# VictoriaMetrics/VictoriaMetrics

Measured on NVIDIA H100. Metric: rollup samples/sec (block decode + rate, raw samples decoded and scanned per second), higher is better.
Workload: dtype int64 codec -> f64 rollup

## Files before the change

victoriametrics_b200/csrc/api.cu:

```cuda
#include <cuda_runtime.h>
#include <cuda_fp16.h>
#include <stdarg.h>
#include <stdio.h>
#include <string.h>
#include <stdlib.h>

#include <algorithm>
#include <vector>

#include "common.cuh"
#include "decode.cu"
#include "rollup.cu"
#include "fused.cu"
#include "zstd.cu"
#include "marshal.inc"
#include "encode.cu"

static thread_local char g_err[512];
void vmb_set_error(const char* fmt, ...) {
    va_list ap;
    va_start(ap, fmt);
    vsnprintf(g_err, sizeof(g_err), fmt, ap);
    va_end(ap);
}
extern "C" const char* vmb_last_error(void) { return g_err; }
extern "C" int vmb_version(void) { return 100; }

#define CU(call)                                                                                   \
    do {                                                                                           \
        cudaError_t e_ = (call);                                                                   \
        if (e_ != cudaSuccess) {                                                                   \
            vmb_set_error("%s failed: %s (%s:%d)", #call, cudaGetErrorString(e_), __FILE__, __LINE__); \
            return VMB_ERR_CUDA;                                                                   \
        }                                                                                          \
    } while (0)

struct DevBuf {
    void* p = nullptr;
    size_t cap = 0;
    int reserve(size_t bytes) {
        if (bytes <= cap) return 0;
        if (p) cudaFree(p);
        p = nullptr;
        cap = 0;
        size_t want = bytes + (bytes >> 3) + 256;
        cudaError_t e = cudaMalloc(&p, want);
        if (e != cudaSuccess) {
            vmb_set_error("cudaMalloc(%zu) failed: %s", want, cudaGetErrorString(e));
            p = nullptr;
            return VMB_ERR_NOMEM;
        }
        cap = want;
        return 0;
    }
    void release() {
        if (p) cudaFree(p);
        p = nullptr;
        cap = 0;
    }
};

enum Stage { ST_ZSTD, ST_DECODE, ST_PREAMBLE, ST_ROLLUP, ST_AGGR, ST_FUSED, ST__COUNT };

#define FUSED_CHUNKS_DEFAULT 4u
#define FUSED_CHUNKS_MAX 64u

struct vmb_ctx {
    int device = 0;
    cudaStream_t stream = 0;
    uint64_t launches = 0;
    bool timing = false;
    float stage_ms[ST__COUNT] = {};
    cudaEvent_t ev[ST__COUNT] = {};
    DevBuf zseq;
    DevBuf zscratch, zlit, zstatus, zjobs, zws, args1, args2, rolled, counters, tmp_out, grp, mheap, mnext;
    DevBuf bail, sub_arrays;
    DevBuf enc_vals, enc_deltas, enc_out, enc_meta;
    DevBuf aggr_state, grp_ids;
    DevBuf oa_keys, oa_keys2, oa_cell, oa_meta;
    DevBuf cv_runs, cv_aux, cv_uniq;
    void* comm = nullptr;
    bool comm_owned = false;
    int comm_ranks = 1, comm_rank = 0;
    bool fused = true;
    uint32_t fused_chunks = 0;
    uint32_t fused_ctas_per_sm = 0;
    cudaStream_t zstream = nullptr;
    std::vector<cudaEvent_t> zev;
    int64_t dedup_interval = 0;
    struct vmb_series* col_cache = nullptr;
    void* h_pinned = nullptr;
    void* pipe = nullptr;
    void (*pipe_destroy)(void*) = nullptr;
};

struct vmb_blocks {
    vmb_ctx* ctx = nullptr;
    size_t nblocks = 0, nseries = 0;
    uint64_t rows = 0, compressed = 0, scratch_total = 0;
    uint64_t merge_rows = 0;
    uint64_t seq_total = 0;
    bool needs_lit = false;
    uint32_t n_huf = 0, n_gen = 0, n_bad = 0;
    uint8_t* d_arrays = nullptr;
    uint64_t* d_ser_merge_off = nullptr;
    vmb_block_desc* d_descs = nullptr;
    uint8_t* d_payload = nullptr;
    uint8_t* d_payload_alloc = nullptr;
    ColInfo* d_cols = nullptr;
    uint64_t* d_row_off = nullptr;
    uint32_t* d_huf_list = nullptr;
    uint32_t* d_gen_list = nullptr;
    uint32_t* d_bad_list = nullptr;
    uint32_t* d_ser_first = nullptr;
    uint32_t* d_ser_nblocks = nullptr;
    uint32_t* d_fused_list = nullptr;
    std::vector<uint32_t> h_fused, h_unfused, h_ser_first, h_ser_nblocks;
    std::vector<uint32_t> h_huf_upto;
    std::vector<vmb_block_desc> h_descs;
    std::vector<ColInfo> h_cols;
};

struct vmb_series {
    vmb_ctx* ctx = nullptr;
    size_t nseries = 0, nblocks = 0;
    uint64_t rows = 0;
    int64_t* d_ts = nullptr;
    double* d_vals = nullptr;
    SeriesMeta* d_meta = nullptr;
    uint32_t* d_blk_lo = nullptr;
    uint32_t* d_blk_hi = nullptr;
    int32_t* d_blk_status = nullptr;
    bool stale_dropped = false, resets_removed = false;
    uint32_t pre_applied = 0;
    bool rolled = false;
    uint32_t applied_mut = 0;
    int64_t applied_max_stale = 0;
    bool values_are_int = false;
};

static inline void count_launch(vmb_ctx* c, int n = 1) { c->launches += (uint64_t)n; }
static inline size_t al16(size_t x) { return (x + 15) & ~(size_t)15; }

extern "C" int vmb_ctx_create(int device, vmb_ctx** out) {
    if (!out) return VMB_ERR_INVALID_ARG;
    int ndev = 0;
    cudaError_t e = cudaGetDeviceCount(&ndev);
    if (e != cudaSuccess || ndev == 0) {
        vmb_set_error("no CUDA device available (%s): libvmb200 has no CPU fallback", cudaGetErrorString(e));
        return VMB_ERR_CUDA;
    }
    if (device < 0 || device >= ndev) {
        vmb_set_error("device %d out of range (%d devices)", device, ndev);
        return VMB_ERR_INVALID_ARG;
    }
    CU(cudaSetDevice(device));
    cudaDeviceProp prop;
    CU(cudaGetDeviceProperties(&prop, device));
    if (prop.major != 9 || prop.minor != 0) {
        vmb_set_error("device %d is sm_%d%d; libvmb200 is built for sm_90a (H100) only", device, prop.major, prop.minor);
        return VMB_ERR_CUDA;
    }
    vmb_ctx* c = new vmb_ctx();
    c->device = device;
    c->fused = getenv("VMB_NO_FUSED") == nullptr;
    if (const char* s = getenv("VMB_FUSED_CHUNKS")) {
        const long v = atol(s);
        c->fused_chunks = v < 1 ? 1u : (v > (long)FUSED_CHUNKS_MAX ? FUSED_CHUNKS_MAX : (uint32_t)v);
    }
    if (const char* s = getenv("VMB_FUSED_CTAS_PER_SM")) {
        const long v = atol(s);
        c->fused_ctas_per_sm = v < 1 ? 1u : (v > FU_CTAS_PER_SM ? (uint32_t)FU_CTAS_PER_SM : (uint32_t)v);
    }
    for (cudaEvent_t& e : c->ev) CU(cudaEventCreate(&e));
    CU(cudaHostAlloc(&c->h_pinned, 4096, cudaHostAllocDefault));
    *out = c;
    return VMB_OK;
}
extern "C" void vmb_series_free(vmb_series* s);
extern "C" int vmb_ctx_comm_destroy(vmb_ctx* ctx);
extern "C" void vmb_ctx_destroy(vmb_ctx* c) {
    if (!c) return;
    cudaSetDevice(c->device);
    cudaStreamSynchronize(c->stream);
    vmb_ctx_comm_destroy(c);
    if (c->col_cache) vmb_series_free(c->col_cache);
    c->col_cache = nullptr;
    DevBuf* bufs[] = {&c->zscratch, &c->zlit, &c->zstatus, &c->zjobs, &c->zws, &c->args1, &c->args2, &c->rolled,
                      &c->counters, &c->tmp_out, &c->grp, &c->mheap, &c->mnext, &c->zseq, &c->bail, &c->sub_arrays, &c->aggr_state, &c->grp_ids, &c->enc_vals, &c->enc_deltas, &c->enc_out, &c->enc_meta,
                      &c->oa_keys, &c->oa_keys2, &c->oa_cell, &c->oa_meta, &c->cv_runs, &c->cv_aux, &c->cv_uniq};
    for (DevBuf* b : bufs) b->release();
    for (cudaEvent_t e : c->ev)
        if (e) cudaEventDestroy(e);
    for (cudaEvent_t e : c->zev) cudaEventDestroy(e);
    if (c->zstream) cudaStreamDestroy(c->zstream);
    if (c->h_pinned) cudaFreeHost(c->h_pinned);
    if (c->pipe && c->pipe_destroy) c->pipe_destroy(c->pipe);
    delete c;
}
extern "C" int vmb_ctx_set_stream(vmb_ctx* c, void* stream) {
    if (!c) return VMB_ERR_INVALID_ARG;
    c->stream = (cudaStream_t)stream;
    return VMB_OK;
}
extern "C" int vmb_ctx_set_dedup_interval(vmb_ctx* c, int64_t interval_ms) {
    if (!c || interval_ms < 0) return VMB_ERR_INVALID_ARG;
    c->dedup_interval = interval_ms;
    return VMB_OK;
}
extern "C" int vmb_ctx_set_fused(vmb_ctx* c, int enable) {
    if (!c) return VMB_ERR_INVALID_ARG;
    c->fused = enable != 0;
    return VMB_OK;
}
extern "C" int vmb_ctx_synchronize(vmb_ctx* c) {
    if (!c) return VMB_ERR_INVALID_ARG;
    CU(cudaSetDevice(c->device));
    CU(cudaStreamSynchronize(c->stream));
    return VMB_OK;
}
extern "C" uint64_t vmb_ctx_launch_count(const vmb_ctx* c) { return c ? c->launches : 0; }
extern "C" float vmb_ctx_last_stage_ms(const vmb_ctx* c, int stage) {
    return (c && stage >= 0 && stage < ST__COUNT) ? c->stage_ms[stage] : 0.f;
}
extern "C" int vmb_ctx_enable_stage_timing(vmb_ctx* c, int enable) {
// ... 395 lines not shown
    for (size_t i = 0; i < nblocks; i++) {
        vmb_block_desc& d = descs[i];
        int rc = vmb_block_desc_from_header(&d, headers + i * 81, tsid);
        if (rc) return rc;
        if (d.ts_off > ts_len || d.ts_size > ts_len - d.ts_off || d.val_off > val_len || d.val_size > val_len - d.val_off) {
            vmb_set_error("block %zu references bytes outside the part files (timestamps [%llu, +%u) of %zu, values [%llu, +%u) of %zu)", i,
                          (unsigned long long)d.ts_off, d.ts_size, ts_len, (unsigned long long)d.val_off, d.val_size, val_len);
            return VMB_ERR_SHORT_SRC;
        }
        if (i && memcmp(tsid, prev_tsid, 24) != 0) series++;
        memcpy(prev_tsid, tsid, 24);
        d.series_idx = series;
        total += al16((size_t)d.ts_size) + al16((size_t)d.val_size);
    }
    std::vector<uint8_t> arena(total + 16);
    size_t pos = 0;
    for (size_t i = 0; i < nblocks; i++) {
        vmb_block_desc& d = descs[i];
        if (d.ts_size) memcpy(arena.data() + pos, timestamps_bin + d.ts_off, d.ts_size);
        d.ts_off = pos;
        pos += al16((size_t)d.ts_size);
        if (d.val_size) memcpy(arena.data() + pos, values_bin + d.val_off, d.val_size);
        d.val_off = pos;
        pos += al16((size_t)d.val_size);
    }
    return blocks_upload_impl(ctx, descs.data(), nblocks, arena.data(), pos, out, 0);
}

extern "C" void vmb_series_free(vmb_series* s) {
    if (!s) return;
    if (s->ctx) cudaSetDevice(s->ctx->device);
    cudaFree(s->d_ts);
    cudaFree(s->d_vals);
    cudaFree(s->d_meta);
    cudaFree(s->d_blk_lo);
    cudaFree(s->d_blk_hi);
    cudaFree(s->d_blk_status);
    delete s;
}
extern "C" size_t vmb_series_count(const vmb_series* s) { return s ? s->nseries : 0; }
extern "C" uint64_t vmb_series_rows(const vmb_series* s) { return s ? s->rows : 0; }

__global__ void k_set_status(int32_t* status, const uint32_t* list, uint32_t n, int32_t v) {
    uint32_t i = blockIdx.x * blockDim.x + threadIdx.x;
    if (i < n) status[list[i]] = v;
}

static void zstd_huf_range(vmb_ctx* ctx, const vmb_blocks* b, ZstdParams Z, uint32_t h0, uint32_t h1, cudaStream_t st) {
    if (h0 >= h1) return;
    Z.jobs = (HufJob*)ctx->zjobs.p + h0;
    Z.list = b->d_huf_list + h0;
    Z.count = h1 - h0;
    launch_zstd_prepare(Z, st);
    launch_huf_decode(Z, st);
    count_launch(ctx, 2);
    if (b->needs_lit) {
        launch_zstd_sequences(Z, st);
        count_launch(ctx, 2);
    }
}

static int run_zstd(vmb_ctx* ctx, const vmb_blocks* b, int32_t** d_zstatus_out, uint32_t huf_end = UINT32_MAX,
                    ZstdParams* Zrest = nullptr) {
    cudaStream_t st = ctx->stream;
    *d_zstatus_out = nullptr;
    if (b->n_huf + b->n_gen + b->n_bad == 0) return VMB_OK;
    int rc;
    if ((rc = ctx->zscratch.reserve(b->scratch_total + 64))) return rc;
    if ((rc = ctx->zstatus.reserve(2 * b->nblocks * sizeof(int32_t)))) return rc;
    int32_t* d_zstatus = (int32_t*)ctx->zstatus.p;
    CU(cudaMemsetAsync(d_zstatus, 0, 2 * b->nblocks * sizeof(int32_t), st));
    if (b->needs_lit && (rc = ctx->zlit.reserve(b->scratch_total + 64))) return rc;
    ZstdParams Z;
    memset(&Z, 0, sizeof(Z));
    Z.descs = b->d_descs;
    Z.cols = b->d_cols;
    Z.payload = b->d_payload;
    Z.scratch = (uint8_t*)ctx->zscratch.p;
    Z.lit = b->needs_lit ? (uint8_t*)ctx->zlit.p : nullptr;
    if (b->seq_total) {
        if ((rc = ctx->zseq.reserve(b->seq_total * 8))) return rc;
        Z.seq_rec = (unsigned long long*)ctx->zseq.p;
    }
    Z.status = d_zstatus;
    if (b->n_bad) {
        k_set_status<<<(b->n_bad + 127) / 128, 128, 0, st>>>(d_zstatus, b->d_bad_list, b->n_bad, VMB_ERR_ZSTD);
        count_launch(ctx);
    }
    const uint32_t ws_threads = VMB_SMS * 2u * 32u;
    if (b->needs_lit || b->n_gen) {
        if ((rc = ctx->zws.reserve((size_t)ws_threads * zstd_serial_ws_bytes()))) return rc;
        Z.ws = ctx->zws.p;
        Z.ws_count = ws_threads;
    }
    if (b->n_huf && (rc = ctx->zjobs.reserve((size_t)b->n_huf * sizeof(HufJob)))) return rc;
    if (Zrest) *Zrest = Z;
    zstd_huf_range(ctx, b, Z, 0, std::min(huf_end, b->n_huf), st);
    if (b->n_gen) {
        Z.list = b->d_gen_list;
        Z.count = b->n_gen;
        launch_zstd_serial(Z, 1, st);
        count_launch(ctx);
    }
    *d_zstatus_out = d_zstatus;
    return VMB_OK;
}

// ... 699 lines not shown
    CU(cudaStreamSynchronize(ctx->stream));
    return VMB_OK;
}

static int column_cache_view(vmb_ctx* ctx, const vmb_blocks* b, vmb_series* view) {
    vmb_series* c = ctx->col_cache;
    if (c && (c->rows < b->rows + b->merge_rows || c->nseries < b->nseries || c->nblocks < b->nblocks)) {
        vmb_series_free(c);
        ctx->col_cache = c = nullptr;
    }
    if (!c) {
        int rc = alloc_series_for(ctx, b, &c);
        if (rc) return rc;
        ctx->col_cache = c;
    }
    *view = *c;
    view->nseries = b->nseries;
    view->nblocks = b->nblocks;
    view->rows = b->rows + b->merge_rows;
    view->stale_dropped = view->resets_removed = view->rolled = false;
    view->pre_applied = 0;
    return 0;
}

static const size_t FUSED_SMEM = (sizeof(FusedSmem) + 15) & ~(size_t)15;
template <typename K>
static uint32_t fused_grid(K kernel) {
    int blocks_per_sm = 0;
    cudaFuncSetAttribute(kernel, cudaFuncAttributeMaxDynamicSharedMemorySize, (int)FUSED_SMEM);
    if (cudaOccupancyMaxActiveBlocksPerMultiprocessor(&blocks_per_sm, kernel, FU_THREADS, FUSED_SMEM) != cudaSuccess || blocks_per_sm < 1)
        blocks_per_sm = 1;
    if (blocks_per_sm > FU_CTAS_PER_SM) blocks_per_sm = FU_CTAS_PER_SM;
    return VMB_SMS * (uint32_t)blocks_per_sm;
}

extern "C" int vmb_fused_grid(void) {
    static const uint32_t grid = fused_grid(k_fused_rollup<VMB_RF_RATE>);
    return (int)grid;
}
extern "C" int vmb_fused_grid_chunked(void) {
    return (int)std::min<uint32_t>((uint32_t)vmb_fused_grid(), VMB_SMS * FU_CTAS_PER_SM_OVERLAP);
}

static uint32_t fused_chunks(const vmb_ctx* ctx, const vmb_blocks* b) {
    const size_t nf = b->h_fused.size();
    uint32_t C = ctx->fused_chunks ? ctx->fused_chunks : FUSED_CHUNKS_DEFAULT;
    if (C > nf) C = (uint32_t)nf;
    if (C <= 1 || b->n_huf == 0) return 1;
    return b->h_huf_upto[nf / C] < b->n_huf ? C : 1u;
}

static uint32_t fused_ctas_per_sm(const vmb_ctx* ctx, uint32_t C, const vmb_rollup_cfg* cfg) {
    if (ctx->fused_ctas_per_sm) return ctx->fused_ctas_per_sm;
    return C > 1 && cfg->func_id == VMB_RF_RATE ? FU_CTAS_PER_SM_OVERLAP : FU_CTAS_PER_SM;
}

static void launch_fused(const FusedParams& P, uint32_t ctas_per_sm, cudaStream_t st) {
    if (!P.nlist) return;
    const size_t smem0 = FUSED_SMEM;
#define FUSED_LAUNCH(KERNEL, SMEM)                                                                                \
    do {                                                                                                          \
        static const uint32_t grid0 = fused_grid(KERNEL);                                                         \
        uint32_t grid = std::min(grid0, VMB_SMS * ctas_per_sm);                                                   \
        if (grid > P.nlist) grid = P.nlist;                                                                       \
        KERNEL<<<grid, FU_THREADS, (SMEM), st>>>(P);                                                              \
    } while (0)
    switch (P.cfg.func_id) {
#define FUSED_CASE(F) case F: FUSED_LAUNCH((k_fused_rollup<F>), smem0); break;
        FUSED_CASE(VMB_RF_RATE)
        FUSED_CASE(VMB_RF_DELTA)
        FUSED_CASE(VMB_RF_AVG)
        FUSED_CASE(VMB_RF_MIN)
        FUSED_CASE(VMB_RF_MAX)
        FUSED_CASE(VMB_RF_SUM)
        FUSED_CASE(VMB_RF_COUNT)
        FUSED_CASE(VMB_RF_QUANTILE)
        FUSED_CASE(VMB_RF_DEFAULT_ROLLUP)
        FUSED_CASE(VMB_RF_IDERIV)
        FUSED_CASE(VMB_RF_IDELTA)
        FUSED_CASE(VMB_RF_LAST)
        FUSED_CASE(VMB_RF_FIRST)
        FUSED_CASE(VMB_RF_STDDEV)
        FUSED_CASE(VMB_RF_STDVAR)
        FUSED_CASE(VMB_RF_CHANGES)
        FUSED_CASE(VMB_RF_DERIV)
#undef FUSED_CASE
        default: FUSED_LAUNCH((k_fused_rollup<-1>), smem0); break;
    }
#undef FUSED_LAUNCH
}

static bool fused_enabled(const vmb_ctx* ctx, const vmb_blocks* b, const vmb_rollup_cfg* cfg) {
    return ctx->fused && !b->h_fused.empty() && ctx->dedup_interval == 0 && !(cfg->flags & VMB_RC_PRE_MASK);
}

static int run_unfused_subset(vmb_ctx* ctx, const vmb_blocks* b, const std::vector<uint32_t>& sub, int32_t* d_zstatus,
                              int64_t tr_min, int64_t tr_max, const vmb_rollup_cfg* cfg, int64_t points, double* d_out,
                              const Counters& c, bool dense_rows) {
    cudaStream_t st = ctx->stream;
    std::vector<vmb_block_desc> descs;
    std::vector<uint32_t> blk_map;
    BlocksPlan pl;
    for (size_t i = 0; i < sub.size(); i++) {
        const uint32_t fb = b->h_ser_first[sub[i]], nb = b->h_ser_nblocks[sub[i]];
        for (uint32_t k = 0; k < nb; k++) {
            vmb_block_desc d = b->h_descs[fb + k];
            d.series_idx = (uint32_t)i;
// ... 401 lines not shown
```

victoriametrics_b200/csrc/zstd.cu:

```cuda
#include "common.cuh"
#include <mutex>

namespace {

__device__ __forceinline__ int hb32(uint32_t v) { return 31 - __clz((int)v); }

struct BitR {
    const uint8_t* base;
    int pos;
    uint64_t buf;
    int cnt;
    long long left;

    __device__ __forceinline__ void refill() {
        uint32_t w;
        if (pos >= 4) {
            w = load_u32_unaligned(base + pos - 4);
            pos -= 4;
        } else {
            w = 0;
            for (int i = 0; i < pos; i++) w |= (uint32_t)base[i] << (8 * i);
            w = pos ? (w << (8 * (4 - pos))) : 0u;
            pos = 0;
        }
// ... 689 lines not shown
        }
        if (hdr + csize >= bsize) break;
        if (regen > ci.content_size) break;
        uint32_t ftab[64];
        short norm[256];
        unsigned short next[256];
        int tlog = 0;
        __align__(16) uint8_t nb_local[256];
        uint32_t used = huf_read_weights(nb_local, &tlog, blk + hdr, csize, ftab, norm, next);
        if (!used) break;
#pragma unroll
        for (int k = 0; k < 32; k++) ((uint64_t*)job->nbits)[k] = ((const uint64_t*)nb_local)[k];
        uint32_t lrem = csize - used;
        const uint8_t* lp = blk + hdr + used;
        if (streams == 1) {
            job->stream_size[0] = lrem;
            job->stream_size[1] = job->stream_size[2] = job->stream_size[3] = 0;
            job->src_off = (uint64_t)(lp - P.payload);
        } else {
            if (lrem < 6) break;
            uint32_t s1 = lp[0] | (lp[1] << 8), s2 = lp[2] | (lp[3] << 8), s3 = lp[4] | (lp[5] << 8);
            if (6 + s1 + s2 + s3 > lrem) break;
            uint32_t seg = (regen + 3) / 4;
            if (seg * 3 > regen) break;
            job->stream_size[0] = s1;
            job->stream_size[1] = s2;
            job->stream_size[2] = s3;
            job->stream_size[3] = lrem - 6 - s1 - s2 - s3;
            job->src_off = (uint64_t)(lp + 6 - P.payload);
        }
        job->regen_size = regen;
        job->table_log = (uint8_t)tlog;
        uint32_t seq_off = hdr + csize;
        job->seq_off = (uint32_t)(blk - src) + seq_off;
        job->seq_size = bsize - seq_off;
        bool has_seq = blk[seq_off] != 0;
        if (!has_seq && (job->seq_size != 1 || regen != ci.content_size)) break;
        if (has_seq && !P.lit) break;
        job->dst_is_lit = has_seq ? 1 : 0;
        job->seq_big = 0;
        job->dst_off = ci.scratch_off;
        job->nstreams = (uint8_t)streams;
        rc = 0;
    } while (0);
    P.status[col] = rc;
}

#define HUF_WARPS 2
#define HUF_FRAMES_PER_WARP 8
#define HUF_MAX_LOG 11
#define HUF_RING 16
#define HUF_FRAME_BYTES (256 + 64)
#define HUF_WARP_TABLE_BYTES (HUF_FRAMES_PER_WARP * HUF_FRAME_BYTES)
#define HUF_FBIAS 0x4B000000u

__global__ void __launch_bounds__(HUF_WARPS * 32) k_huf_decode(ZstdParams P) {
    extern __shared__ __align__(16) uint8_t s_smem[];
    const int lane = lane_id();
    const int warp = threadIdx.x >> 5;
    const uint32_t groups = (P.count + HUF_FRAMES_PER_WARP - 1) / HUF_FRAMES_PER_WARP;
    uint8_t* wtab = s_smem + (size_t)warp * HUF_WARP_TABLE_BYTES;
    uint32_t* wring = (uint32_t*)(s_smem + (size_t)HUF_WARPS * HUF_WARP_TABLE_BYTES) + (size_t)warp * HUF_RING * 32;
    for (uint32_t g = blockIdx.x * HUF_WARPS + warp; g < groups; g += gridDim.x * HUF_WARPS) {
        for (int f = 0; f < HUF_FRAMES_PER_WARP; f++) {
            uint32_t ji = g * HUF_FRAMES_PER_WARP + f;
            if (ji >= P.count) break;
            const HufJob* job = &P.jobs[ji];
            if (job->nstreams == 0) continue;
            const int log = job->table_log;
            uint8_t* perm = wtab + f * HUF_FRAME_BYTES;
            float* thr = (float*)(perm + 256);
            short* adj = (short*)(perm + 256 + 40);
            uint32_t nb[8];
            uint64_t packed = *(const uint64_t*)(job->nbits + lane * 8);
#pragma unroll
            for (int k = 0; k < 8; k++) nb[k] = (uint32_t)(packed >> (8 * k)) & 0xff;
            uint32_t start = 0;
            uint32_t rank = 0;
            if (lane < 10) thr[lane] = __uint_as_float(HUF_FBIAS);
            __syncwarp();
            for (int len = log; len >= 1; len--) {
                uint32_t mine = 0;
#pragma unroll
                for (int k = 0; k < 8; k++) mine += (nb[k] == (uint32_t)len);
                uint32_t inc = mine;
#pragma unroll
                for (int off = 1; off < 32; off <<= 1) {
                    uint32_t t = __shfl_up_sync(VMB_FULL, inc, off);
                    if (lane >= off) inc += t;
                }
                uint32_t tot = __shfl_sync(VMB_FULL, inc, 31);
                if (lane == 0) {
                    if (len <= 10) thr[len - 1] = __uint_as_float(HUF_FBIAS | start);
                    adj[len] = (short)((int)rank - (int)(start >> (HUF_MAX_LOG - len)));
                }
                uint32_t r = rank + inc - mine;
#pragma unroll
                for (int k = 0; k < 8; k++) {
                    if (nb[k] == (uint32_t)len) perm[r++ & 255u] = (uint8_t)(lane * 8 + k);
                }
                rank += tot;
                start += tot << (HUF_MAX_LOG - len);
            }
        }
        __syncwarp();
        {
            const int f = lane >> 2, s = lane & 3;
            uint32_t ji = g * HUF_FRAMES_PER_WARP + f;
            bool active = ji < P.count;
            const HufJob* job = active ? &P.jobs[ji] : nullptr;
            if (active && (job->nstreams == 0 || s >= job->nstreams)) active = false;
            bool ok = true;
            if (active) {
                const uint8_t* perm = wtab + f * HUF_FRAME_BYTES;
                const short* adj = (const short*)(perm + 256 + 40);
                __half2 th2[5];
                {
                    const float* tf = (const float*)(perm + 256);
#pragma unroll
                    for (int j = 0; j < 5; j++) {
                        const uint32_t a = __float_as_uint(tf[2 * j]) & 0x7fffffu, b = __float_as_uint(tf[2 * j + 1]) & 0x7fffffu;
                        th2[j] = __halves2half2(__ushort2half_rn((unsigned short)a), __ushort2half_rn((unsigned short)b));
                    }
                }
                uint32_t regen = job->regen_size;
                uint32_t seg = job->nstreams == 1 ? regen : (regen + 3) / 4;
                uint32_t count = job->nstreams == 1 ? regen : (s < 3 ? seg : regen - 3 * seg);
                uint64_t soff = job->src_off;
                for (int k = 0; k < s; k++) soff += job->stream_size[k];
                uint32_t slen = job->stream_size[s];
                uint8_t* dst = (job->dst_is_lit ? P.lit : P.scratch) + job->dst_off + (size_t)s * seg;
                const uint8_t* base = P.payload + soff;
                uint32_t last = slen ? base[slen - 1] : 0;
                if (count == 0) {
                } else if (slen == 0 || last == 0) {
                    ok = false;
                } else {
                    const uint32_t total_bits = (slen - 1) * 8 + (uint32_t)hb32(last);
                    const uint8_t* endp = base + slen - 1;
                    const uint4* blk = (const uint4*)((uintptr_t)endp & ~(uintptr_t)15);
                    const uint4* blk_min = (const uint4*)(((uintptr_t)base & ~(uintptr_t)15) - 32);
                    uint32_t* ring = wring + lane;
                    uint32_t wr = 0, rd = 0;
                    uint64_t buf;
                    int cnt;
                    {
                        uint4 q = *blk;
                        uint64_t qlo = ((uint64_t)q.y << 32) | q.x, qhi = ((uint64_t)q.w << 32) | q.z;
                        uint32_t nbytes = (uint32_t)((uintptr_t)endp & 15) + 1;
                        uint32_t drop = (16 - nbytes) * 8;
                        if (drop >= 64) { qhi = qlo; qlo = 0; drop -= 64; }
                        if (drop) { qhi = (qhi << drop) | (qlo >> (64 - drop)); qlo <<= drop; }
                        uint32_t r = nbytes & 3;
                        if (r == 0) r = 4;
                        buf = qhi & ~(~0ull >> (8 * r));
                        cnt = (int)(8 * r);
                        qhi = (qhi << (8 * r)) | (r == 8 ? 0 : (qlo >> (64 - 8 * r)));
                        qlo <<= (8 * r);
                        uint32_t nw = (nbytes - r) >> 2;
                        for (uint32_t k = 0; k < nw; k++) {
                            ring[(wr & (HUF_RING - 1)) * 32] = (uint32_t)(qhi >> 32);
                            wr++;
                            qhi = (qhi << 32) | (qlo >> 32);
                            qlo <<= 32;
                        }
                        int skip = 8 - hb32(last);
                        buf <<= skip;
                        cnt -= skip;
#pragma unroll
                        for (int k = 0; k < 3; k++) {
                            if (blk > blk_min) blk--;
                            uint4 b = *blk;
                            ring[((wr + 0) & (HUF_RING - 1)) * 32] = b.w;
                            ring[((wr + 1) & (HUF_RING - 1)) * 32] = b.z;
                            ring[((wr + 2) & (HUF_RING - 1)) * 32] = b.y;
                            ring[((wr + 3) & (HUF_RING - 1)) * 32] = b.x;
                            wr += 4;
                        }
                    }
                    const int cnt_init = cnt;
                    uint4 pendA = make_uint4(0, 0, 0, 0), pendB = make_uint4(0, 0, 0, 0);
                    bool hasA = false, hasB = false;
                    uint32_t cand = ring[(rd & (HUF_RING - 1)) * 32];
#define HUF_PHASE(pend, has)                                                               \
    do {                                                                                   \
        if (has) {            \
            ring[((wr + 0) & (HUF_RING - 1)) * 32] = pend.w;                               \
            ring[((wr + 1) & (HUF_RING - 1)) * 32] = pend.z;                               \
            ring[((wr + 2) & (HUF_RING - 1)) * 32] = pend.y;                               \
            ring[((wr + 3) & (HUF_RING - 1)) * 32] = pend.x;                               \
            wr += 4;                                                                       \
        }                                                                                  \
                   \
        has = (wr - rd) + 8u <= (uint32_t)HUF_RING;                                        \
        if (has) {                                                                         \
            if (blk > blk_min) blk--;                                                      \
            pend = *blk;                                                                   \
        }                                                                                  \
        cand = ring[(rd & (HUF_RING - 1)) * 32];  \
    } while (0)
#define HUF_REFILL()                                                                       \
    do {                                                                                   \
        if (cnt <= 32) {                                                                   \
            buf |= (uint64_t)cand << (32 - cnt);                                           \
            cnt += 32;                                                                     \
            rd++;                                                                          \
        }                                                                                  \
        cand = ring[(rd & (HUF_RING - 1)) * 32];                                           \
    } while (0)
#define HUF_LT(k) __hlt2(vv_, th2[k])
#define HUF_SYM(outv, shift)                                                               \
    do {                                                                                   \
        const uint32_t v_ = (uint32_t)(buf >> 53);                                         \
        const __half2 vv_ = __half2half2(__ushort2half_rn((unsigned short)v_));            \
                  \
        const __half2 c_ = __hadd2(__hadd2(__hadd2(HUF_LT(0), HUF_LT(1)), __hadd2(HUF_LT(2), HUF_LT(3))), HUF_LT(4)); \
        const uint32_t nb_ = 1u + (uint32_t)__half2ushort_rz(__hadd(__low2half(c_), __high2half(c_))); \
        buf <<= nb_;                                                                       \
        cnt -= (int)nb_;                                                                   \
        const uint32_t sym_ = perm[((v_ >> (HUF_MAX_LOG - nb_)) + (uint32_t)(int)adj[nb_]) & 255u]; \
        outv |= sym_ << (shift);                                                           \
    } while (0)
                    uint32_t i = 0;
                    while (i < count && (((uintptr_t)(dst + i)) & 15)) {
                        HUF_REFILL();
                        uint32_t o = 0;
                        HUF_SYM(o, 0);
                        dst[i++] = (uint8_t)o;
                    }
                    for (; i + 16 <= count; i += 16) {
                        uint32_t o[4];
                        HUF_PHASE(pendA, hasA);
#pragma unroll
                        for (int q = 0; q < 2; q++) {
                            o[q] = 0;
                            HUF_REFILL();
                            HUF_SYM(o[q], 0);
                            HUF_SYM(o[q], 8);
                            HUF_REFILL();
                            HUF_SYM(o[q], 16);
                            HUF_SYM(o[q], 24);
                        }
                        HUF_PHASE(pendB, hasB);
#pragma unroll
                        for (int q = 2; q < 4; q++) {
                            o[q] = 0;
                            HUF_REFILL();
                            HUF_SYM(o[q], 0);
                            HUF_SYM(o[q], 8);
                            HUF_REFILL();
                            HUF_SYM(o[q], 16);
                            HUF_SYM(o[q], 24);
                        }
                        *(uint4*)(dst + i) = make_uint4(o[0], o[1], o[2], o[3]);
                    }
                    if (i < count) {
                        HUF_PHASE(pendA, hasA);
                        HUF_PHASE(pendB, hasB);
                        hasA = hasB = false;
                    }
                    for (; i < count; i++) {
                        HUF_REFILL();
                        uint32_t o = 0;
                        HUF_SYM(o, 0);
                        dst[i] = (uint8_t)o;
                    }
#undef HUF_PHASE
#undef HUF_REFILL
#undef HUF_SYM
#undef HUF_LT
                    ok = (long long)cnt_init + 32ll * (long long)rd - (long long)cnt == (long long)total_bits;
                }
            }
            uint32_t bad = __ballot_sync(VMB_FULL, active && !ok);
            if (ji < P.count && s == 0 && ((bad >> (f * 4)) & 0xf)) P.status[P.jobs[ji].col] = VMB_ERR_ZSTD;
        }
        __syncwarp();
    }
}

#define SEQ_G 4
#define SEQ_FPW (32 / SEQ_G)
#define SEQ_WARPS 1
#define SEQ_REC(ll, ml, of) (((unsigned long long)(ll) << 44) | ((unsigned long long)(ml) << 24) | (unsigned long long)(of))
#define SEQ_REC_LL(r) ((uint32_t)((r) >> 44))
#define SEQ_REC_ML(r) ((uint32_t)((r) >> 24) & 0xfffffu)
#define SEQ_REC_OF(r) ((uint32_t)(r) & 0xffffffu)
template <int LLC, int MLC, int OFC>
struct SeqTablesT {
    unsigned short ll_nb[LLC], ml_nb[MLC], of_nb[OFC];
    uint8_t ll_sym[LLC], ml_sym[MLC], of_sym[OFC];
};

__device__ bool fse_build_packed(uint8_t* sym, unsigned short* nbbase, const short* norm, int nsym, int log, unsigned short* next) {
    const int size = 1 << log;
    int high = size - 1;
    for (int s = 0; s < nsym; s++) {
        if (norm[s] == -1) {
            sym[high--] = (uint8_t)s;
            next[s] = 1;
        } else {
            next[s] = (unsigned short)norm[s];
        }
    }
    const int step = (size >> 1) + (size >> 3) + 3, mask = size - 1;
    int pos = 0;
    for (int s = 0; s < nsym; s++) {
        for (int i = 0; i < norm[s]; i++) {
            sym[pos] = (uint8_t)s;
            do {
                pos = (pos + step) & mask;
            } while (pos > high);
        }
    }
    if (pos != 0) return false;
    for (int i = 0; i < size; i++) {
        const uint32_t s = sym[i];
        const uint32_t ns = next[s]++;
        const int nb = log - hb32(ns);
        nbbase[i] = (unsigned short)(((uint32_t)nb << 12) | ((ns << nb) - (uint32_t)size));
    }
    return true;
}

#define SEQ_DEF_LL 0
#define SEQ_DEF_OF 64
#define SEQ_DEF_ML 96
__device__ unsigned short g_seq_def_nb[160];
__device__ uint8_t g_seq_def_sym[160];
__global__ void k_zstd_seq_defaults() {
    if (blockIdx.x || threadIdx.x) return;
// ... 372 lines not shown
                __syncwarp();
            }
            o_base += __shfl_sync(VMB_FULL, so, 31);
            l_base += __shfl_sync(VMB_FULL, sl, 31);
        }
        warp_copy(out + o_base, lits + l_base, job->regen_size - l_base, lane);
        __syncwarp();
    }
}

__global__ void k_zstd_serial(ZstdParams P, int mode) {
    uint32_t tid = blockIdx.x * blockDim.x + threadIdx.x;
    if (tid >= P.ws_count) return;
    SerialWs* ws = (SerialWs*)P.ws + tid;
    for (uint32_t i = tid; i < P.count; i += P.ws_count) {
        if (mode == 0) {
            const HufJob* job = &P.jobs[i];
            if (job->nstreams == 0 || !job->dst_is_lit) continue;
            uint32_t col = job->col;
            if (P.status[col]) continue;
            const ColInfo ci = P.cols[col];
            const uint8_t* src;
            uint32_t len;
            col_src(P, col, &src, &len);
            ws->have_ll = ws->have_ml = ws->have_of = 0;
            ws->rep[0] = 1;
            ws->rep[1] = 4;
            ws->rep[2] = 8;
            long long o = run_sequences(ws, P.scratch + ci.scratch_off, 0, ci.content_size, P.lit + ci.scratch_off,
                                        job->regen_size, src + job->seq_off, job->seq_size);
            if (o != (long long)ci.content_size) P.status[col] = VMB_ERR_ZSTD;
        } else {
            uint32_t col = P.list[i];
            const ColInfo ci = P.cols[col];
            const uint8_t* src;
            uint32_t len;
            col_src(P, col, &src, &len);
            const long long o = P.lit ? decode_frame_serial(ws, P.scratch + ci.scratch_off, ci.content_size,
                                                            P.lit + ci.scratch_off, src, len)
                                      : -1;
            P.status[col] = o >= 0 ? 0 : VMB_ERR_ZSTD;
            if (o >= 0 && o != (long long)ci.content_size) P.cols[col].content_size = (uint32_t)o;
        }
    }
}

size_t zstd_serial_ws_bytes() { return sizeof(SerialWs); }

void launch_zstd_prepare(const ZstdParams& P, cudaStream_t st) {
    if (!P.count) return;
    k_zstd_prepare<<<(P.count + 63) / 64, 64, 0, st>>>(P);
}

void launch_huf_decode(const ZstdParams& P, cudaStream_t st) {
    if (!P.count) return;
    constexpr size_t smem = (size_t)HUF_WARPS * HUF_WARP_TABLE_BYTES + (size_t)HUF_WARPS * HUF_RING * 32 * sizeof(uint32_t);
    static_assert(smem <= 48 * 1024, "k_huf_decode would need cudaFuncAttributeMaxDynamicSharedMemorySize");
    uint32_t groups = (P.count + HUF_FRAMES_PER_WARP - 1) / HUF_FRAMES_PER_WARP;
    uint32_t grid = (groups + HUF_WARPS - 1) / HUF_WARPS;
    if (grid > VMB_SMS * 12u) grid = VMB_SMS * 12u;
    k_huf_decode<<<grid, HUF_WARPS * 32, smem, st>>>(P);
}

void launch_zstd_sequences(const ZstdParams& P, cudaStream_t st) {
    if (!P.count || !P.ws_count || !P.seq_rec) return;
    const uint32_t per_cta = SEQ_WARPS * SEQ_FPW;
    const uint64_t slots = (uint64_t)P.ws_count * sizeof(SerialWs) / sizeof(SeqWs);
    uint64_t groups = P.count < slots ? P.count : slots;
    uint32_t grid = (uint32_t)((groups + per_cta - 1) / per_cta);
    if ((uint64_t)grid * per_cta > slots) grid = (uint32_t)(slots / per_cta);
    if (grid == 0) grid = 1;
    {
        static std::mutex mu;
        static bool built[64] = {};
        int dev = 0;
        cudaGetDevice(&dev);
        std::lock_guard<std::mutex> lk(mu);
        if (!built[dev & 63]) {
            k_zstd_seq_defaults<<<1, 32, 0, st>>>();
            if (cudaStreamSynchronize(st) == cudaSuccess) built[dev & 63] = true;
        }
    }
    k_zstd_seq_decode<false><<<grid, SEQ_WARPS * 32, 0, st>>>(P);
    k_zstd_seq_decode<true><<<grid, SEQ_WARPS * 32, 0, st>>>(P);
    uint32_t xgrid = (P.count + SEQX_WARPS - 1) / SEQX_WARPS;
    if (xgrid > VMB_SMS * 64u) xgrid = VMB_SMS * 64u;
    k_zstd_seq_exec<<<xgrid, SEQX_WARPS * 32, 0, st>>>(P);
}

void launch_zstd_serial(const ZstdParams& P, int mode, cudaStream_t st) {
    if (!P.count || !P.ws_count) return;
    uint32_t threads = P.ws_count < P.count ? P.ws_count : P.count;
    k_zstd_serial<<<(threads + 31) / 32, 32, 0, st>>>(P, mode);
}


static bool zstd_content_bound_host(const FrameHdr& h, const uint8_t* src, uint32_t len, unsigned long long* bound) {
    unsigned long long b = 0;
    uint32_t pos = h.hdr_size;
    for (;;) {
        if (pos + 3 > len) return false;
        const uint32_t bh = src[pos] | ((uint32_t)src[pos + 1] << 8) | ((uint32_t)src[pos + 2] << 16);
        pos += 3;
        const uint32_t bsize = bh >> 3, type = (bh >> 1) & 3;
        if (type == 3) return false;
        const uint32_t stored = type == 1 ? 1u : bsize;
        if ((unsigned long long)pos + stored > len) return false;
        pos += stored;
        b += type == 2 ? h.block_max : bsize;
        if (bh & 1) break;
    }
    *bound = b;
    return true;
}

// ... 66 lines not shown
```

Baseline: 61.96 billion.

## Stage Huffman decode output in shared memory for coalesced warp stores

The Huffman decode body now writes each lane's 16-byte output chunks into a per-warp shared-memory staging ring. When the ring fills, the warp cooperatively flushes it so consecutive lanes write consecutive 16-byte pieces of the same stream, instead of each lane scattering its own uint4 stores. The change also lowers the default fused chunk count from 4 to 2, always uses the normal fused CTAs-per-SM, and adds an env knob for Huffman CTAs per SM. Compile-time experiment flags (phase timers, L1 no-allocate loads, integer threshold compare) are added but off by default. The cost is more shared memory per CTA and extra warp votes and shuffles in the loop.

```diff
diff --git a/victoriametrics_b200/csrc/api.cu b/victoriametrics_b200/csrc/api.cu
--- a/victoriametrics_b200/csrc/api.cu
+++ b/victoriametrics_b200/csrc/api.cu
@@ -62,7 +62,7 @@
 
 enum Stage { ST_ZSTD, ST_DECODE, ST_PREAMBLE, ST_ROLLUP, ST_AGGR, ST_FUSED, ST__COUNT };
 
-#define FUSED_CHUNKS_DEFAULT 4u
+#define FUSED_CHUNKS_DEFAULT 2u
 #define FUSED_CHUNKS_MAX 64u
 
 struct vmb_ctx {
@@ -85,6 +85,7 @@
     bool fused = true;
     uint32_t fused_chunks = 0;
     uint32_t fused_ctas_per_sm = 0;
+    uint32_t huf_ctas_per_sm = 0;
     cudaStream_t zstream = nullptr;
     std::vector<cudaEvent_t> zev;
     int64_t dedup_interval = 0;
@@ -171,6 +172,10 @@
     if (const char* s = getenv("VMB_FUSED_CTAS_PER_SM")) {
         const long v = atol(s);
         c->fused_ctas_per_sm = v < 1 ? 1u : (v > FU_CTAS_PER_SM ? (uint32_t)FU_CTAS_PER_SM : (uint32_t)v);
+    }
+    if (const char* s = getenv("VMB_HUF_CTAS_PER_SM")) {
+        const long v = atol(s);
+        c->huf_ctas_per_sm = v < 1 ? 1u : (v > 32 ? 32u : (uint32_t)v);
     }
     for (cudaEvent_t& e : c->ev) CU(cudaEventCreate(&e));
     CU(cudaHostAlloc(&c->h_pinned, 4096, cudaHostAllocDefault));
@@ -672,7 +677,7 @@
     Z.list = b->d_huf_list + h0;
     Z.count = h1 - h0;
     launch_zstd_prepare(Z, st);
-    launch_huf_decode(Z, st);
+    launch_huf_decode(Z, ctx->huf_ctas_per_sm, st);
     count_launch(ctx, 2);
     if (b->needs_lit) {
         launch_zstd_sequences(Z, st);
@@ -1478,7 +1483,9 @@
 
 static uint32_t fused_ctas_per_sm(const vmb_ctx* ctx, uint32_t C, const vmb_rollup_cfg* cfg) {
     if (ctx->fused_ctas_per_sm) return ctx->fused_ctas_per_sm;
-    return C > 1 && cfg->func_id == VMB_RF_RATE ? FU_CTAS_PER_SM_OVERLAP : FU_CTAS_PER_SM;
+    (void)C;
+    (void)cfg;
+    return FU_CTAS_PER_SM;
 }
 
 static void launch_fused(const FusedParams& P, uint32_t ctas_per_sm, cudaStream_t st) {
diff --git a/victoriametrics_b200/csrc/zstd.cu b/victoriametrics_b200/csrc/zstd.cu
--- a/victoriametrics_b200/csrc/zstd.cu
+++ b/victoriametrics_b200/csrc/zstd.cu
@@ -765,7 +765,49 @@
 #define HUF_RING 16
 #define HUF_FRAME_BYTES (256 + 64)
 #define HUF_WARP_TABLE_BYTES (HUF_FRAMES_PER_WARP * HUF_FRAME_BYTES)
+#ifndef HUF_STAGE
+#define HUF_STAGE 8
+#endif
+#define HUF_STAGE_SLOT(q, l) ((q) * 32 + ((l) ^ ((q) * (8 / HUF_STAGE))))
 #define HUF_FBIAS 0x4B000000u
+#define HUF_CTAS_PER_SM 12u
+
+#ifndef VMB_HUF_EXP
+#define VMB_HUF_EXP 0
+#endif
+#define HUF_EXP_STORE 1
+#define HUF_EXP_LOOKUP 2
+#define HUF_EXP_CONVERT 4
+#define HUF_EXP_INPUT 8
+#define HUF_EXP_L1 16
+#define HUF_EXP_PHASES 32
+#define HUF_EXP_CARVEOUT 64
+#define HUF_EXP(bit) ((VMB_HUF_EXP & (bit)) != 0)
+enum { HUF_PH_BUILD, HUF_PH_PRIME, HUF_PH_HEAD, HUF_PH_BODY, HUF_PH_TAIL, HUF_PH_N, HUF_PH_SYMS = HUF_PH_N, HUF_PH_SLOTS };
+#if HUF_EXP(HUF_EXP_PHASES)
+__device__ unsigned long long huf_phase_cyc[HUF_PH_SLOTS];
+#define HUF_PH(k)                                                                              \
+    do {                                                                                       \
+        const long long ph_c = clock64();                                                      \
+        ph[(k)] += (unsigned long long)(ph_c - ph_t);                                          \
+        ph_t = ph_c;                                                                           \
+    } while (0)
+#else
+#define HUF_PH(k) \
+    do {          \
+    } while (0)
+#endif
+
+__device__ __forceinline__ uint4 huf_ldg(const uint4* p) {
+    if (HUF_EXP(HUF_EXP_L1)) {
+        uint4 r;
+        asm volatile("ld.global.nc.L1::no_allocate.v4.u32 {%0,%1,%2,%3}, [%4];"
+                     : "=r"(r.x), "=r"(r.y), "=r"(r.z), "=r"(r.w)
+                     : "l"(p));
+        return r;
+    }
+    return *p;
+}
 
 __global__ void __launch_bounds__(HUF_WARPS * 32) k_huf_decode(ZstdParams P) {
     extern __shared__ __align__(16) uint8_t s_smem[];
@@ -774,6 +816,10 @@
     const uint32_t groups = (P.count + HUF_FRAMES_PER_WARP - 1) / HUF_FRAMES_PER_WARP;
     uint8_t* wtab = s_smem + (size_t)warp * HUF_WARP_TABLE_BYTES;
     uint32_t* wring = (uint32_t*)(s_smem + (size_t)HUF_WARPS * HUF_WARP_TABLE_BYTES) + (size_t)warp * HUF_RING * 32;
+#if HUF_EXP(HUF_EXP_PHASES)
+    unsigned long long ph[HUF_PH_SLOTS] = {};
+    long long ph_t = clock64();
+#endif
     for (uint32_t g = blockIdx.x * HUF_WARPS + warp; g < groups; g += gridDim.x * HUF_WARPS) {
         for (int f = 0; f < HUF_FRAMES_PER_WARP; f++) {
             uint32_t ji = g * HUF_FRAMES_PER_WARP + f;
@@ -817,6 +863,7 @@
             }
         }
         __syncwarp();
+        HUF_PH(HUF_PH_BUILD);
         {
             const int f = lane >> 2, s = lane & 3;
             uint32_t ji = g * HUF_FRAMES_PER_WARP + f;
@@ -824,10 +871,22 @@
             const HufJob* job = active ? &P.jobs[ji] : nullptr;
             if (active && (job->nstreams == 0 || s >= job->nstreams)) active = false;
             bool ok = true;
+            bool live = false;
+            const uint8_t* perm = wtab + f * HUF_FRAME_BYTES;
+            const short* adj = (const short*)(perm + 256 + 40);
+            __half2 th2[5];
+            uint32_t th_i[5] = {0, 0, 0, 0, 0};
+            uint32_t count = 0, total_bits = 0, wr = 0, rd = 0, cand = 0, i = 0;
+            uint8_t* dst = nullptr;
+            const uint4* blk = nullptr;
+            const uint4* blk_min = nullptr;
+            uint32_t* ring = wring + lane;
+            uint64_t buf = 0;
+            int cnt = 0, cnt_init = 0;
+            uint4 pendA = make_uint4(0, 0, 0, 0), pendB = make_uint4(0, 0, 0, 0);
+            bool hasA = false, hasB = false;
+            uint4 xo = make_uint4(0, 0, 0, 0);
             if (active) {
-                const uint8_t* perm = wtab + f * HUF_FRAME_BYTES;
-                const short* adj = (const short*)(perm + 256 + 40);
-                __half2 th2[5];
                 {
                     const float* tf = (const float*)(perm + 256);
 #pragma unroll
@@ -836,27 +895,31 @@
                         th2[j] = __halves2half2(__ushort2half_rn((unsigned short)a), __ushort2half_rn((unsigned short)b));
                     }
                 }
+                if (HUF_EXP(HUF_EXP_CONVERT)) {
+                    const float* tf = (const float*)(perm + 256);
+#pragma unroll
+                    for (int j = 0; j < 5; j++)
+                        th_i[j] = ((0x1000u + (__float_as_uint(tf[2 * j + 1]) & 0x7fffffu)) << 16) |
+                                  (0x1000u + (__float_as_uint(tf[2 * j]) & 0x7fffffu));
+                }
                 uint32_t regen = job->regen_size;
                 uint32_t seg = job->nstreams == 1 ? regen : (regen + 3) / 4;
-                uint32_t count = job->nstreams == 1 ? regen : (s < 3 ? seg : regen - 3 * seg);
+                count = job->nstreams == 1 ? regen : (s < 3 ? seg : regen - 3 * seg);
                 uint64_t soff = job->src_off;
                 for (int k = 0; k < s; k++) soff += job->stream_size[k];
                 uint32_t slen = job->stream_size[s];
-                uint8_t* dst = (job->dst_is_lit ? P.lit : P.scratch) + job->dst_off + (size_t)s * seg;
+                dst = (job->dst_is_lit ? P.lit : P.scratch) + job->dst_off + (size_t)s * seg;
                 const uint8_t* base = P.payload + soff;
                 uint32_t last = slen ? base[slen - 1] : 0;
                 if (count == 0) {
                 } else if (slen == 0 || last == 0) {
                     ok = false;
                 } else {
-                    const uint32_t total_bits = (slen - 1) * 8 + (uint32_t)hb32(last);
+                    live = true;
+                    total_bits = (slen - 1) * 8 + (uint32_t)hb32(last);
                     const uint8_t* endp = base + slen - 1;
-                    const uint4* blk = (const uint4*)((uintptr_t)endp & ~(uintptr_t)15);
-                    const uint4* blk_min = (const uint4*)(((uintptr_t)base & ~(uintptr_t)15) - 32);
-                    uint32_t* ring = wring + lane;
-                    uint32_t wr = 0, rd = 0;
-                    uint64_t buf;
-                    int cnt;
+                    blk = (const uint4*)((uintptr_t)endp & ~(uintptr_t)15);
+                    blk_min = (const uint4*)(((uintptr_t)base & ~(uintptr_t)15) - 32);
                     {
                         uint4 q = *blk;
                         uint64_t qlo = ((uint64_t)q.y << 32) | q.x, qhi = ((uint64_t)q.w << 32) | q.z;
@@ -883,7 +946,7 @@
 #pragma unroll
                         for (int k = 0; k < 3; k++) {
                             if (blk > blk_min) blk--;
-                            uint4 b = *blk;
+                            uint4 b = huf_ldg(blk);
                             ring[((wr + 0) & (HUF_RING - 1)) * 32] = b.w;
                             ring[((wr + 1) & (HUF_RING - 1)) * 32] = b.z;
                             ring[((wr + 2) & (HUF_RING - 1)) * 32] = b.y;
@@ -891,10 +954,8 @@
                             wr += 4;
                         }
                     }
-                    const int cnt_init = cnt;
-                    uint4 pendA = make_uint4(0, 0, 0, 0), pendB = make_uint4(0, 0, 0, 0);
-                    bool hasA = false, hasB = false;
-                    uint32_t cand = ring[(rd & (HUF_RING - 1)) * 32];
+                    cnt_init = cnt;
+                    cand = ring[(rd & (HUF_RING - 1)) * 32];
 #define HUF_PHASE(pend, has)                                                               \
     do {                                                                                   \
         if (has) {            \
@@ -908,7 +969,8 @@
         has = (wr - rd) + 8u <= (uint32_t)HUF_RING;                                        \
         if (has) {                                                                         \
             if (blk > blk_min) blk--;                                                      \
-            pend = *blk;                                                                   \
+            if (HUF_EXP(HUF_EXP_INPUT)) pend = make_uint4(rd, wr, (uint32_t)cnt, (uint32_t)(uintptr_t)blk); \
+            else pend = huf_ldg(blk);                                                      \
         }                                                                                  \
         cand = ring[(rd & (HUF_RING - 1)) * 32];  \
     } while (0)
@@ -922,26 +984,44 @@
         cand = ring[(rd & (HUF_RING - 1)) * 32];                                           \
     } while (0)
 #define HUF_LT(k) __hlt2(vv_, th2[k])
+#define HUF_LTI(j) ((th_i[j] - v1_) & 0x10001000u)
 #define HUF_SYM(outv, shift)                                                               \
     do {                                                                                   \
         const uint32_t v_ = (uint32_t)(buf >> 53);                                         \
-        const __half2 vv_ = __half2half2(__ushort2half_rn((unsigned short)v_));            \
+        uint32_t nb_;                                                                      \
+        if (HUF_EXP(HUF_EXP_CONVERT)) {                                                    \
+            const uint32_t v1_ = (v_ + 1u) * 0x10001u;                                     \
+            const uint32_t a_ = HUF_LTI(0) + HUF_LTI(1) + HUF_LTI(2) + HUF_LTI(3) + HUF_LTI(4); \
+            nb_ = 1u + ((a_ * 0x10001u) >> 28);                                            \
+        } else {                                                                           \
+            const __half2 vv_ = __half2half2(__ushort2half_rn((unsigned short)v_));        \
                   \
-        const __half2 c_ = __hadd2(__hadd2(__hadd2(HUF_LT(0), HUF_LT(1)), __hadd2(HUF_LT(2), HUF_LT(3))), HUF_LT(4)); \
-        const uint32_t nb_ = 1u + (uint32_t)__half2ushort_rz(__hadd(__low2half(c_), __high2half(c_))); \
+            const __half2 c_ = __hadd2(__hadd2(__hadd2(HUF_LT(0), HUF_LT(1)), __hadd2(HUF_LT(2), HUF_LT(3))), HUF_LT(4)); \
+            nb_ = 1u + (uint32_t)__half2ushort_rz(__hadd(__low2half(c_), __high2half(c_))); \
+        }                                                                                  \
         buf <<= nb_;                                                                       \
         cnt -= (int)nb_;                                                                   \
-        const uint32_t sym_ = perm[((v_ >> (HUF_MAX_LOG - nb_)) + (uint32_t)(int)adj[nb_]) & 255u]; \
+        const uint32_t sym_ = HUF_EXP(HUF_EXP_LOOKUP) ? ((v_ >> (HUF_MAX_LOG - nb_)) & 255u)  \
+            : perm[((v_ >> (HUF_MAX_LOG - nb_)) + (uint32_t)(int)adj[nb_]) & 255u];         \
         outv |= sym_ << (shift);                                                           \
     } while (0)
-                    uint32_t i = 0;
+                    HUF_PH(HUF_PH_PRIME);
                     while (i < count && (((uintptr_t)(dst + i)) & 15)) {
                         HUF_REFILL();
                         uint32_t o = 0;
                         HUF_SYM(o, 0);
                         dst[i++] = (uint8_t)o;
                     }
-                    for (; i + 16 <= count; i += 16) {
+                    HUF_PH(HUF_PH_HEAD);
+                }
+            }
+            {
+                uint4* stage = (uint4*)(s_smem + (size_t)HUF_WARPS * (HUF_WARP_TABLE_BYTES + HUF_RING * 32 * sizeof(uint32_t))) +
+                               warp * HUF_STAGE * 32;
+                uint32_t k = 0, bi = i;
+                for (;;) {
+                    const bool more = live && i + 16 <= count;
+                    if (more) {
                         uint32_t o[4];
                         HUF_PHASE(pendA, hasA);
 #pragma unroll
@@ -965,8 +1045,36 @@
                             HUF_SYM(o[q], 16);
                             HUF_SYM(o[q], 24);
                         }
-                        *(uint4*)(dst + i) = make_uint4(o[0], o[1], o[2], o[3]);
+                        if (HUF_EXP(HUF_EXP_STORE)) {
+                            xo.x ^= o[0]; xo.y ^= o[1]; xo.z ^= o[2]; xo.w ^= o[3];
+                        } else {
+                            stage[HUF_STAGE_SLOT(k, lane)] = make_uint4(o[0], o[1], o[2], o[3]);
+                        }
+                        i += 16;
                     }
+                    const bool any = __any_sync(VMB_FULL, more);
+                    if (++k == HUF_STAGE || !any) {
+                        __syncwarp();
+                        const uint32_t n_l = (i - bi) >> 4;
+                        const uintptr_t p_l = (uintptr_t)(dst + bi);
+#pragma unroll
+                        for (int j = 0; j < HUF_STAGE; j++) {
+                            const int l = (j * 32 + lane) / HUF_STAGE, q = (j * 32 + lane) % HUF_STAGE;
+                            const uint32_t n = __shfl_sync(VMB_FULL, n_l, l);
+                            const uintptr_t pp = (uintptr_t)__shfl_sync(VMB_FULL, (unsigned long long)p_l, l);
+                            if ((uint32_t)q < n && !HUF_EXP(HUF_EXP_STORE)) *(uint4*)(pp + 16 * q) = stage[HUF_STAGE_SLOT(q, l)];
+                        }
+                        __syncwarp();
+                        k = 0;
+                        bi = i;
+                    }
+                    if (!any) break;
+                }
+            }
+            if (HUF_EXP(HUF_EXP_STORE) && live && i >= 16) *(uint4*)(dst + i - 16) = xo;
+            if (live) {
+                {
+                    HUF_PH(HUF_PH_BODY);
                     if (i < count) {
                         HUF_PHASE(pendA, hasA);
                         HUF_PHASE(pendB, hasB);
@@ -978,18 +1086,29 @@
                         HUF_SYM(o, 0);
                         dst[i] = (uint8_t)o;
                     }
+                    HUF_PH(HUF_PH_TAIL);
+#if HUF_EXP(HUF_EXP_PHASES)
+                    ph[HUF_PH_SYMS] += count;
+#endif
 #undef HUF_PHASE
 #undef HUF_REFILL
 #undef HUF_SYM
 #undef HUF_LT
+#undef HUF_LTI
                     ok = (long long)cnt_init + 32ll * (long long)rd - (long long)cnt == (long long)total_bits;
                 }
             }
+            if (HUF_EXP(HUF_EXP_STORE | HUF_EXP_LOOKUP | HUF_EXP_INPUT)) ok = false;
             uint32_t bad = __ballot_sync(VMB_FULL, active && !ok);
+            if (HUF_EXP(HUF_EXP_STORE | HUF_EXP_LOOKUP | HUF_EXP_INPUT) && ji < P.count && s == 0) bad |= 1u << (f * 4);
             if (ji < P.count && s == 0 && ((bad >> (f * 4)) & 0xf)) P.status[P.jobs[ji].col] = VMB_ERR_ZSTD;
         }
         __syncwarp();
     }
+#if HUF_EXP(HUF_EXP_PHASES)
+    if (lane == 0)
+        for (int k = 0; k < HUF_PH_SLOTS; k++) atomicAdd(&huf_phase_cyc[k], ph[k]);
+#endif
 }
 
 #define SEQ_G 4
@@ -1468,15 +1587,32 @@
     k_zstd_prepare<<<(P.count + 63) / 64, 64, 0, st>>>(P);
 }
 
-void launch_huf_decode(const ZstdParams& P, cudaStream_t st) {
+void launch_huf_decode(const ZstdParams& P, uint32_t ctas_per_sm, cudaStream_t st) {
     if (!P.count) return;
-    constexpr size_t smem = (size_t)HUF_WARPS * HUF_WARP_TABLE_BYTES + (size_t)HUF_WARPS * HUF_RING * 32 * sizeof(uint32_t);
+    constexpr size_t smem = (size_t)HUF_WARPS * HUF_WARP_TABLE_BYTES + (size_t)HUF_WARPS * HUF_RING * 32 * sizeof(uint32_t) +
+                            (size_t)HUF_WARPS * HUF_STAGE * 32 * sizeof(uint4);
     static_assert(smem <= 48 * 1024, "k_huf_decode would need cudaFuncAttributeMaxDynamicSharedMemorySize");
+    const uint32_t cap = ctas_per_sm ? ctas_per_sm : HUF_CTAS_PER_SM;
+    if (HUF_EXP(HUF_EXP_CARVEOUT)) {
+        const int pct = (int)((cap * (smem + 1024) * 100 + 228 * 1024 - 1) / (228 * 1024));
+        cudaFuncSetAttribute(k_huf_decode, cudaFuncAttributePreferredSharedMemoryCarveout, pct > 100 ? 100 : pct);
+    }
     uint32_t groups = (P.count + HUF_FRAMES_PER_WARP - 1) / HUF_FRAMES_PER_WARP;
     uint32_t grid = (groups + HUF_WARPS - 1) / HUF_WARPS;
-    if (grid > VMB_SMS * 12u) grid = VMB_SMS * 12u;
+    if (grid > VMB_SMS * cap) grid = VMB_SMS * cap;
     k_huf_decode<<<grid, HUF_WARPS * 32, smem, st>>>(P);
 }
+
+#if HUF_EXP(HUF_EXP_PHASES)
+extern "C" int vmb_huf_phase_cycles(unsigned long long* out, int reset) {
+    if (out && cudaMemcpyFromSymbol(out, huf_phase_cyc, sizeof(huf_phase_cyc)) != cudaSuccess) return -1;
+    if (reset) {
+        static const unsigned long long zero[HUF_PH_SLOTS] = {};
+        if (cudaMemcpyToSymbol(huf_phase_cyc, zero, sizeof(zero)) != cudaSuccess) return -1;
+    }
+    return HUF_PH_SLOTS;
+}
+#endif
 
 void launch_zstd_sequences(const ZstdParams& P, cudaStream_t st) {
     if (!P.count || !P.ws_count || !P.seq_rec) return;
```

New measurement: 66.00 billion (median of 6 runs). 1.07x the previous value.
